# aperezhortal/pySPEEDY

Hardware: AMD Instinct MI355X
Metric: simulated-years/day (whole node), T30L8 (higher is better)
Workload: dtype f64

## Files before the change

### pyspeedy_amd/csrc/dyn_column.hpp

```cpp
#pragma once
#include <hip/hip_runtime.h>

#include "model.hpp"
#include "stream_store.hpp"
#include "vertical_consts.hpp"

namespace spd {

struct NoPrefetch {
    __device__ void operator()() const {}
};
template <bool STORE_ALL, typename F = NoPrefetch>
__device__ __forceinline__ void dyn_column(const ModelPtrs &P, const DynDeviceTables &D, int mem, int p, int j,
                                           double (&ttend)[KX], double (&trtend)[KX], double &utend_kx, double &vtend_kx,
                                           F before_products = F{}) {
    constexpr int NG = IX * IL;
    constexpr double AKAPd = 2.0f / 7.0f, RGASd = AKAPd * static_cast<double>(1004.0f);
    const size_t o3 = static_cast<size_t>(mem) * KX * NG + p, o2 = static_cast<size_t>(mem) * NG + p;
    double ug[KX], vg[KX], tg[KX], trg[KX], vorg[KX], divg[KX];
    const double cor = D.coriol[j];
#pragma unroll
    for (int k = 0; k < KX; ++k) {
        ug[k] = stream_load(&P.ug2[o3 + NG * k]);
        vg[k] = stream_load(&P.vg2[o3 + NG * k]);
        tg[k] = stream_load(&P.tg2[o3 + NG * k]);
        trg[k] = stream_load(&P.trg2[o3 + NG * k]);
        vorg[k] = stream_load(&P.vorg[o3 + NG * k]);
        divg[k] = stream_load(&P.divg[o3 + NG * k]);
    }
    const double px = stream_load(&P.px[o2]), py = stream_load(&P.py[o2]);
    __builtin_amdgcn_sched_barrier(0);
#pragma unroll
    for (int k = 0; k < KX; ++k) vorg[k] = vorg[k] + cor;
    double umean = 0.0, vmean = 0.0, dmean = 0.0;
#pragma unroll
    for (int k = 0; k < KX; ++k) {
// ... 20 lines not shown
    for (int k = 1; k < KX; ++k) temp[k] = sigdt[k] * (ug[k] - ug[k - 1]);
#pragma unroll
    for (int k = 0; k < KX; ++k) {
        const double v = vg[k] * vorg[k] - tgg[k] * RGASd * px - (temp[k + 1] + temp[k]) * vc::dhsr[k];
        if (STORE_ALL || k < KX - 1) stream_store(&P.utend[o3 + NG * k], v);
        if (k == KX - 1) utend_kx = v;
    }
#pragma unroll
    for (int k = 1; k < KX; ++k) temp[k] = sigdt[k] * (vg[k] - vg[k - 1]);
#pragma unroll
    for (int k = 0; k < KX; ++k) {
        const double v = -ug[k] * vorg[k] - tgg[k] * RGASd * py - (temp[k + 1] + temp[k]) * vc::dhsr[k];
        if (STORE_ALL || k < KX - 1) stream_store(&P.vtend[o3 + NG * k], v);
        if (k == KX - 1) vtend_kx = v;
    }
#pragma unroll
    for (int k = 1; k < KX; ++k) temp[k] = sigdt[k] * (tgg[k] - tgg[k - 1]) + sigm[k] * (vc::tref[k] - vc::tref[k - 1]);
#pragma unroll
    for (int k = 0; k < KX; ++k) {
        ttend[k] = tgg[k] * divg[k] - (temp[k + 1] + temp[k]) * vc::dhsr[k] + vc::fsgr[k] * tgg[k] * (sigdt[k + 1] + sigdt[k]) +
                   vc::tref3[k] * (sigm[k + 1] + sigm[k]) + AKAPd * (tg[k] * puv[k] - tgg[k] * dmean);
        if (STORE_ALL) stream_store(&P.ttend[o3 + NG * k], ttend[k]);
    }
#pragma unroll
    for (int k = 1; k < KX; ++k) temp[k] = sigdt[k] * (trg[k] - trg[k - 1]);
    temp[1] = 0.0;
    temp[2] = 0.0;
#pragma unroll
    for (int k = 0; k < KX; ++k) {
        trtend[k] = trg[k] * divg[k] - (temp[k + 1] + temp[k]) * vc::dhsr[k];
        if (STORE_ALL) stream_store(&P.trtend[o3 + NG * k], trtend[k]);
    }
    before_products();
#pragma unroll
    for (int k = 0; k < KX; ++k) {
        stream_store(&P.keg[o3 + NG * k], 0.5f * (ug[k] * ug[k] + vg[k] * vg[k]));
        stream_store(&P.utg[o3 + NG * k], -ug[k] * tgg[k]);
        stream_store(&P.vtg[o3 + NG * k], -vg[k] * tgg[k]);
        stream_store(&P.uqg[o3 + NG * k], -ug[k] * trg[k]);
        stream_store(&P.vqg[o3 + NG * k], -vg[k] * trg[k]);
    }
}

}
```

### pyspeedy_amd/csrc/model.hip

```cpp
#include <dlfcn.h>
#include <hip/hip_runtime.h>

#include <algorithm>
#include <atomic>
#include <chrono>
#include <cmath>
#include <cstring>
#include <map>
#include <memory>
#include <mutex>
#include <string>
#include <thread>
#include <utility>
#include <vector>

#include "model_state.hpp"
#include "coupler_point.hpp"
#include "diagnostics_block.hpp"
#include "bounded_call.hpp"
#include "launch_events.hpp"
#include "sppt_point.hpp"
#include "stream_apart.hpp"

namespace spd {
hipError_t run_spec2grid_table(const DeviceTables &T, const FieldDesc *table, int nfields, hipStream_t st);
hipError_t run_grid2spec_table(const DeviceTables &T, const FieldDesc *table, int nfields, hipStream_t st);
hipError_t run_physics(const DeviceTables &T, const spd_physics_args &a, int nmembers, int fp32, hipStream_t s);
hipError_t run_dyn_physics(const ModelPtrs &P, const DynDeviceTables &D, const DeviceTables &T, const spd_physics_args &a,
                           int first, int nmembers, int fp32, int store32, int diag, hipStream_t s);
hipError_t run_geopotential(const ModelPtrs &P, const DynDeviceTables &D, int first, int count, int tl, const SpptArgs *sppt,
                            int *rim, hipStream_t s);
hipError_t run_dyn_grid(const ModelPtrs &P, const DynDeviceTables &D, int M, hipStream_t s);
hipError_t run_spectral_step(const ModelPtrs &P, const DeviceTables &T, const DynDeviceTables &D, int M, int first, int count,
                             int j1, double dt, double eps, const CouplerArgs *cpl, bool early, int rim_mode, int *rim, hipStream_t s);
hipError_t run_diagnostics(const ModelPtrs &P, const DeviceTables &T, int M, int tl, int *err, double *diag, int ticket,
                           hipStream_t s);
hipError_t run_diagnostics_range(const ModelPtrs &P, const DeviceTables &T, int first, int count, int tl, int *err, double *diag,
                                 int ticket, hipStream_t s);
hipError_t run_coupler(const SurfacePtrs &S, int first, int count, const TimeInterp &w, int day, int land_coupling,
                       int sst_anomaly, int anom_planes, int fresh, hipStream_t s);
hipError_t run_forcing(const SurfacePtrs &S, int first, int count, const ZonalDevice &Z, double gamlat, double *corh_t,
                       double *corh_q, hipStream_t s);
hipError_t run_rest_state(const RestPtrs &R, int M, const RestConsts &c, hipStream_t s);
hipError_t run_scale_orog(const double *orog, double *phi0, long n, hipStream_t s);
hipError_t run_change_storage(double *array, long n, bool to_float, void *scratch, hipStream_t s);
hipError_t run_land_sea_init(const LandSeaPtrs &P, const LandSeaConsts &K, int first, int count, double *rows, hipStream_t s);
hipError_t run_multi_copy(const CopyList &L, hipStream_t s);
hipError_t run_spec2grid_table_check(const DeviceTables &T, const FieldDesc *table, int nfields, const CheckArgs &check, int members,
                                     hipStream_t st);
hipError_t run_copy_from_first(double *v, long n, int M, const int *flags, hipStream_t s);
hipError_t run_rest_surface(const double *phis0, double *forog, double *surf_ps, double *surf_q, const RestConsts &c, long n,
                            hipStream_t s);
hipError_t run_grid2spec(const DeviceTables &T, int stage, const double *src, double *dst, int prescale, int nfields,
                         hipStream_t stream);
// ... 143 lines not shown
    if (!m->inv_table32[0][0]) build_inverse_tables(m, false, true, m->inv_table32, batch);
    if (m->sppt_spec && !m->inv_table_sppt32[0][0]) build_inverse_tables(m, true, true, m->inv_table_sppt32, batch);
    return batch.upload(m);
}

static int build_tables(spd_model *m) {
    const int M = m->M;
    const ModelPtrs &P = m->P;
    auto spec = [](double *base, size_t field) { return base + field * NSPEC * C; };
    auto grid = [](double *base, size_t field) { return base + field * NG; };
    TableBatch batch;
    build_inverse_tables(m, false, false, m->inv_table, batch);
    auto pspec = [](double *base, size_t field) { return base + field * tri::kPacked * C; };
    constexpr int pk = kSpecPacked;
    std::vector<FieldDesc> t;
    t.reserve(static_cast<size_t>(M) * 73);
    const size_t pair = static_cast<size_t>(M) * 8;
    for (int i = 0; i < M; ++i) {
        const size_t w = static_cast<size_t>(i) * 8;
        for (int k = 0; k < 8; ++k) {
            t.push_back({grid(P.utend, w + k), pspec(P.specu, w + k), 1 | pk, 0});
            t.push_back({grid(P.vtend, w + k), pspec(P.specv, w + k), 1 | pk, 0});
            t.push_back({grid(P.utg, w + k), pspec(P.specu, pair + w + k), 1 | pk, 0});
            t.push_back({grid(P.vtg, w + k), pspec(P.specv, pair + w + k), 1 | pk, 0});
            t.push_back({grid(P.uqg, w + k), pspec(P.specu, 2 * pair + w + k), 1 | pk, 0});
            t.push_back({grid(P.vqg, w + k), pspec(P.specv, 2 * pair + w + k), 1 | pk, 0});
            t.push_back({grid(P.ttend, w + k), pspec(P.spec_tt, w + k), pk, 0});
            t.push_back({grid(P.trtend, w + k), pspec(P.spec_tr, w + k), pk, 0});
            t.push_back({grid(P.keg, w + k), pspec(P.spec_ke, w + k), pk, 0});
        }
        t.push_back({grid(P.psdtg, i), pspec(P.spec_ps, i), pk, 0});
    }
    batch.add(std::move(t), &m->fwd_table);
    for (int par = 0; par < 2; ++par) {
        std::vector<FieldDesc> ti, tf;
        const size_t half = static_cast<size_t>(M) * 16;
        for (int i = 0; i < M; ++i) {
            const size_t w = static_cast<size_t>(i) * 8, s1 = static_cast<size_t>(i) * 16;
            for (int k = 0; k < 8; ++k) {
                ti.push_back({spec(P.sv, s1 + k), grid(m->u_grid, w + k), 2, 0});
                ti.push_back({spec(P.sv, half + s1 + k), grid(m->v_grid, w + k), 2, 0});
                ti.push_back({spec(P.t, s1 + k), grid(m->t_grid, w + k), 1, 0});
                ti.push_back({spec(P.tr, s1 + k), grid(m->q_grid, w + k), 1, 0});
                ti.push_back({spec(m->phi_buf[par], w + k), grid(m->phi_grid, w + k), 1, 0});
                tf.push_back({grid(m->u_grid, w + k), spec(P.sv, s1 + k), 1, 0});
                tf.push_back({grid(m->v_grid, w + k), spec(P.sv, half + s1 + k), 1, 0});
                tf.push_back({grid(m->t_grid, w + k), spec(P.t, s1 + k), 0, 0});
                tf.push_back({grid(m->q_grid, w + k), spec(P.tr, s1 + k), 0, 0});
                tf.push_back({grid(m->phi_grid, w + k), spec(m->phi_buf[par], w + k), 0, 0});
            }
            ti.push_back({spec(P.ps, static_cast<size_t>(i) * 2), grid(m->ps_grid, i), 1, 0});
        }
        batch.add(std::move(ti), &m->exp_inv_table[par]);
        batch.add(std::move(tf), &m->exp_fwd_table[par]);
    }
    return batch.upload(m);
}

namespace spd {
int sample_ids(const char *who, const char *const *names, int n_names, std::vector<int> &ids) {
    if (n_names < 0 || (n_names > 0 && !names)) return m_fail(SPD_E_ARG, std::string(who) + ": bad list of variable names");
    for (int k = 0; k < n_names; ++k) {
        const int id = names[k] ? stats_id(names[k]) : -1;
        if (id < 0)
            return m_fail(SPD_E_ARG, std::string(who) + ": unknown variable '" + (names[k] ? names[k] : "(null)") +
                                         "' (u_grid, v_grid, t_grid, q_grid, phi_grid, ps_grid, precnv, precls, u_plev, v_plev, t_plev, "
// ... 514 lines not shown
        else (void)hipEventRecord(start, s);
    }
    ~ProfScope() {
        if (!stop) return;
        if (!attach) {
            (void)hipEventRecord(stop, s);
        } else if (pending_launch_events().start == start) {
            pending_launch_events() = LaunchEvents{};
            (void)hipEventRecord(start, s);
            (void)hipEventRecord(stop, s);
        }
    }
};

static bool folds(const spd_model *m) { return m->fold_geo && !m->nudge.loops(); }

static bool begin_step_geopotential(spd_model *m) {
    const bool fold = folds(m);
    const bool ahead = fold && m->phi_ahead;
    if (ahead) m->phi_cur ^= 1;
    m->P.phi = m->phi_buf[m->phi_cur];
    m->P.phi_next = fold ? m->phi_buf[m->phi_cur ^ 1] : nullptr;
    m->reg["phi"].ptr = m->P.phi;
    m->phi_ahead = fold;
    return !ahead;
}

static void sppt_advance(spd_model *m) {
    if (!m->sppt_on) return;
    m->sppt_first = false;
    m->sppt_step += 1;
}

static hipError_t step_range(spd_model *m, int j1, int j2, double dt, int compute_shortwave, int first, int count, int diag,
                             bool run_geo, const CouplerArgs *cpl, hipStream_t s, hipEvent_t after_grid2spec = nullptr,
                             const CheckArgs *ride = nullptr, int rim_mode = kRimPlain) {
    const DeviceTables &T = m->ctx->dev;
    const int M = m->M;
    hipError_t e = hipSuccess;
    if (m->fail_launch_after >= 0 && m->fail_launch_after-- == 0) return hipErrorLaunchFailure;
    SpptArgs sp{};
    if (m->sppt_on)
        sp = sppt_args(m->sppt_spec + static_cast<size_t>(first) * 8 * NSPEC * C, T, count, m->sppt_seed, m->sppt_member_base + first,
                       m->sppt_step, m->sppt_first ? 1 : 0);
    if (run_geo) {
        ProfScope ps(m, SPD_K_GEOPOTENTIAL, count, s);
        e = run_geopotential(m->P, m->D, first, count, 0, m->sppt_on ? &sp : nullptr, rim_mode == kRimSkip ? m->d_rim : nullptr,
                             s);
    } else if (m->sppt_on) {
        ProfScope ps(m, SPD_K_SPPT, 8 * count, s);
        e = run_sppt_update(sp, s);
    }
    spd_physics_args pa = m->pa;
    pa.compute_shortwave = compute_shortwave ? 1 : 0;
    pa.air_absortivity_co2 = m->air_absortivity_co2;
    pa.sppt_pattern = m->sppt_on ? m->sppt_grid : nullptr;
    if (e == hipSuccess) {
        const int per = m->inv_per_member + (m->sppt_on ? 8 : 0);
        FieldDesc *table = (m->stored32 ? (m->sppt_on ? m->inv_table_sppt32 : m->inv_table32)
                                         : (m->sppt_on ? m->inv_table_sppt : m->inv_table))[j2 - 1][m->phi_cur];
        ProfScope ps(m, SPD_K_SPEC2GRID, per * count, s);
        if (m->deferred.active && first == 0 && count == M && s == m->deferred.stream) {
            const int slot = m->deferred.slot;
            const CheckArgs chk{m->P.vor, m->P.div, m->P.t, m->deferred.time_level - 1, m->h_err[slot], m->d_diag, m->slot_ticket[slot]};
            e = run_spec2grid_table_check(T, table, per * count, chk, M, s);
            m->deferred.active = false;
            m->slot_rode[slot] = true;
            ++m->checks_rode;
        } else if (ride) {
            e = run_spec2grid_table_check(T, table + static_cast<size_t>(first) * per, per * count, *ride, count, s);
            ++m->checks_rode;
        } else {
            e = run_spec2grid_table(T, table + static_cast<size_t>(first) * per, per * count, s);
        }
    }
    if (e == hipSuccess) {
        if (m->split_dyn_physics && !m->phys_fp32) {
            {
                ProfScope ps(m, SPD_K_DYN_GRID, M, s);
                e = run_dyn_grid(m->P, m->D, M, s);
            }
            if (e == hipSuccess) {
                ProfScope ps(m, compute_shortwave ? SPD_K_PHYSICS_SW : SPD_K_PHYSICS, M, s);
                e = run_physics(T, pa, M, m->phys_fp32, s);
            }
        } else {
            ProfScope ps(m, compute_shortwave ? SPD_K_COLUMN_SW : SPD_K_COLUMN, count, s);
            e = run_dyn_physics(m->P, m->D, T, pa, first, count, m->phys_fp32, m->stored32 ? 1 : 0, diag, s);
        }
    }
    if (e == hipSuccess) {
        ProfScope ps(m, SPD_K_GRID2SPEC, 73 * count, s);
        e = run_grid2spec_table(T, m->fwd_table + static_cast<size_t>(first) * 73, 73 * count, s);
    }
    if (after_grid2spec && e == hipSuccess) e = hipEventRecord(after_grid2spec, s);
    const double eps = (j1 == 1) ? 0.0 : static_cast<double>(0.05f);
    if (e == hipSuccess) {
        ProfScope ps(m, SPD_K_SPECTRAL_STEP, count, s);
        const bool early = m->spectral_early < 0 ? count <= 8 : m->spectral_early != 0;
        e = run_spectral_step(m->P, T, m->D, M, first, count, j1 - 1, dt, eps, cpl, early, rim_mode, m->d_rim, s);
    }
    return e;
}

int spd_model_step_dynamics(spd_model_handle m, int j1, int j2, double dt, int compute_shortwave, void *stream) {
    if (!m) return m_fail(SPD_E_ARG, "spd_model_step_dynamics: null model");
    if (j1 < 1 || j1 > 2 || j2 < 1 || j2 > 2) return m_fail(SPD_E_ARG, "spd_model_step_dynamics: time levels are 1 or 2");
    if (!m->dyn) return m_fail(SPD_E_ARG, "spd_model_step_dynamics: call spd_model_set_time_step first");
    if (int rc = settle_deferred_check(m)) return rc;
    const bool run_geo = begin_step_geopotential(m);
    const hipError_t e = step_range(m, j1, j2, dt, compute_shortwave, 0, m->M, 1, run_geo, nullptr, static_cast<hipStream_t>(stream));
    if (e != hipSuccess) return m_fail(SPD_E_DEVICE, std::string("spd_model_step_dynamics: ") + hipGetErrorString(e));
    sppt_advance(m);
    return SPD_OK;
}

static int next_ticket(spd_model *m) {
    m->check_ticket = m->check_ticket % 0x0fffffff + 1;
    return m->check_ticket;
}

static int wait_codes(spd_model *m, const int *pinned, int ticket, hipEvent_t ev, hipStream_t s, int32_t *out, const char *who) {
    const volatile int *codes = pinned;
    const int M = m->M;
    auto all_there = [&]() {
        for (int i = 0; i < M; ++i)
// ... 798 lines not shown
        const long n = static_cast<long>(kv.second.bytes_member / sizeof(double)) * m->M;
        e = run_change_storage(static_cast<double *>(kv.second.ptr), n, fp32 != 0, scratch, nullptr);
        ++converted;
    }
    if (e == hipSuccess) e = hipDeviceSynchronize();
    (void)hipFree(scratch);
    if (e != hipSuccess) {
        if (converted > 0) {
            m->initialized = false;
            m->poisoned = std::string("a device error (") + hipGetErrorString(e) + ") interrupted the change of its fp32 / fp64 storage; "
                          "create and initialise a new model";
        }
        return m_fail(SPD_E_DEVICE, std::string("spd_model_set_physics_precision: ") + hipGetErrorString(e));
    }
    m->stored32 = want32;
    return SPD_OK;
}

int spd_model_set_physics_precision(spd_model_handle m, int fp32) {
    if (!m) return m_fail(SPD_E_ARG, "spd_model_set_physics_precision: null model");
    m->phys_fp32 = fp32 ? 1 : 0;
    return apply_storage(m, m->phys_fp32 && m->phys_store32);
}

int spd_model_get_option(spd_model_handle m, const char *name, int32_t *value) {
    if (!m || !name || !value) return m_fail(SPD_E_ARG, "spd_model_get_option: null argument");
    const std::string key(name);
    if (key == "diag_every_step") *value = m->diag_every_step ? 1 : 0;
    else if (key == "split_dyn") *value = m->split_dyn_physics ? 1 : 0;
    else if (key == "spectral_early") *value = m->spectral_early;
    else if (key == "member_groups") *value = m->nchunks;
    else if (key == "block_members") *value = m->block_members;
    else if (key == "physics_storage32") *value = m->phys_store32 ? 1 : 0;
    else if (key == "quiet_rim_members") {
        *value = -1;
        if (m->rim_call) {
            std::vector<int> flags(static_cast<size_t>(m->M));
            M_HIP(hipDeviceSynchronize());
            M_HIP(hipMemcpy(flags.data(), m->d_rim, sizeof(int) * flags.size(), hipMemcpyDeviceToHost));
            *value = 0;
            for (int f : flags) *value += f != 0 ? 1 : 0;
        }
    }
    else return m_fail(SPD_E_ARG, "spd_model_get_option: unknown option: " + key);
    return SPD_OK;
}

int spd_model_set_option(spd_model_handle m, const char *name, int32_t value) {
    if (!m || !name) return m_fail(SPD_E_ARG, "spd_model_set_option: null argument");
    const std::string key(name);
    const bool flag = value == 0 || value == 1;
    if (key == "diag_every_step" && flag) m->diag_every_step = value != 0;
    else if (key == "split_dyn" && flag) m->split_dyn_physics = value != 0;
    else if (key == "spectral_early" && value >= -1 && value <= 1) m->spectral_early = value;
    else if (key == "member_groups" && value >= 1 && value <= 4) m->nchunks = value < m->M ? value : m->M;
    else if (key == "block_members" && value >= 0) m->block_members = value;
    else if (key == "fail_launch_after" && value >= -1) m->fail_launch_after = value;
    else if (key == "prepare_multi_step" && value == 1) {
        if (int rc = ensure_steps_record(m, 360)) return rc;
        if (m->nchunks > 1 && !m->split_dyn_physics) return ensure_group_streams(m, m->nchunks);
    }
    else if (key == "physics_storage32" && flag) {
        m->phys_store32 = value != 0;
        return apply_storage(m, m->phys_fp32 && m->phys_store32);
    }
    else return m_fail(SPD_E_ARG, "spd_model_set_option: unknown option or value out of range: " + key);
// ... 366 lines not shown
```

### pyspeedy_amd/csrc/model_state.hpp

```cpp
#pragma once
#include <hip/hip_runtime.h>

#include <algorithm>
#include <cmath>
#include <cstring>
#include <map>
#include <memory>
#include <string>
#include <utility>
#include <vector>

#include "../../include/pyspeedy_amd.h"
#include "context.hpp"
#include "model.hpp"
#include "plev.hpp"
#include "stats.hpp"
#include "spectra.hpp"
#include "tape.hpp"
#include "enstape.hpp"
#include "acctape.hpp"
#include "nudge.hpp"
#include "breed.hpp"
#include "wintape.hpp"
#include "projtape.hpp"
// ... 1 lines not shown
#include "surface.hpp"

using namespace spd;

namespace spd {
constexpr int NG = IX * IL;
constexpr size_t C = 2;

struct RegEntry {
    void *ptr;
    size_t bytes_member;
    bool f32 = false;
};
}

struct spd_model {
    spd_context *ctx = nullptr;
    int M = 0;
    ModelPtrs P{};
    const spd_dyn_tables *dyn = nullptr;
    std::unique_ptr<spd_dyn_tables> dyn_private;
    DynDeviceTables D{};
    spd_physics_args pa{};
    struct Block {
        char *base;
        size_t size, used;
    };
    std::vector<Block> blocks;
    std::map<std::string, RegEntry> reg;
    FieldDesc *inv_table[2][2] = {{nullptr, nullptr}, {nullptr, nullptr}};
    FieldDesc *inv_table_sppt[2][2] = {{nullptr, nullptr}, {nullptr, nullptr}};
    FieldDesc *inv_table32[2][2] = {{nullptr, nullptr}, {nullptr, nullptr}}, *inv_table_sppt32[2][2] = {{nullptr, nullptr}, {nullptr, nullptr}};
    FieldDesc *fwd_table = nullptr;
    double *phi_buf[2] = {nullptr, nullptr};
    int phi_cur = 0;
    bool phi_ahead = false, fold_geo = true;
    bool groups_apart = true;
    int *d_err = nullptr;
    double *d_diag = nullptr;
    int *d_rim = nullptr;
    bool rim_call = false;
    int *h_err[2] = {nullptr, nullptr}, *h_err_sync = nullptr;
    hipEvent_t err_event[2] = {nullptr, nullptr};
    int next_slot = 0;
    bool slot_busy[2] = {false, false};
    int check_ticket = 0, slot_ticket[2] = {0, 0};
    struct DeferredCheck {
        bool active = false;
        int slot = -1, time_level = 2;
        hipStream_t stream = nullptr;
    } deferred;
    hipStream_t slot_stream[2] = {nullptr, nullptr};
    bool slot_rode[2] = {false, false};
    int checks_alone = 0, checks_rode = 0;
    double air_absortivity_co2 = 6.0;
    SurfacePtrs S{};
    Calendar cal;
    int current_step = 0;
    bool initialized = false;
    bool sppt_on = false, sppt_first = true;
    unsigned long long sppt_seed = 0;
    long long sppt_member_base = 0, sppt_step = 0;
    double *sppt_spec = nullptr, *sppt_grid = nullptr;
    int inv_per_member = 77;
    int nchunks = 1;
    int block_members = 32;
// ... 296 lines not shown
```

### pyspeedy_amd/csrc/transforms.hip

```cpp
#include <hip/hip_runtime.h>

#include "device_tables.hpp"
#include "diagnostics_block.hpp"
#include "launch_events.hpp"
#include "fft96.hpp"
#include "triangle.hpp"

namespace spd {

constexpr int kThreads = 512;
constexpr int kRowStride = 97;
constexpr int kRows = IL;
constexpr int kCStride = 63;
constexpr int kCBufDoubles = kRows * kCStride;
constexpr int kSpecPerLane = (NSPEC + kThreads - 1) / kThreads;
constexpr int kGridPerLane = (NGRID / 2 + kThreads - 1) / kThreads;
constexpr int kPlanePerLane = (kRows * MX + kThreads - 1) / kThreads;
constexpr int kHalfPlanePerLane = (IY * MX + kThreads - 1) / kThreads;
constexpr int kInvLanes = MX * 12;
constexpr size_t kLdsBytes = (kCBufDoubles + 2 * NSPEC) * sizeof(double);
static_assert(kRows * kRowStride <= kCBufDoubles + 2 * NSPEC, "R must fit inside C + S");

enum class Stage { Fused, LegendreOnly, FourierOnly };

using d2 = double __attribute__((ext_vector_type(2)));
using gd2_in = const __attribute__((address_space(1))) d2 *;
using gd2_out = __attribute__((address_space(1))) d2 *;
typedef float f2 __attribute__((ext_vector_type(2)));
using gf2_out = __attribute__((address_space(1))) f2 *;

__device__ inline int pos_re(int m) { return m == 0 ? 0 : 2 * m - 1; }
__device__ inline int pos_im(int m) { return m == 0 ? 61 : 2 * m; }

__device__ inline int wave_id() { return __builtin_amdgcn_readfirstlane(static_cast<int>(threadIdx.x) >> 6); }

#ifdef SPD_TRACE
__device__ unsigned long long spd_trace_acc[2][8];
__device__ unsigned long long spd_trace_cnt[2];
#define TRACE_BEGIN() unsigned long long trace_t0 = (threadIdx.x == 0) ? wall_clock64() : 0ull
// ... 168 lines not shown

    const bool as_float = (kcos & kGridAsFloat) != 0;
    kcos &= ~kGridAsFloat;
    gd2_out g = (gd2_out)dst;
    double cs[kGridPerLane];
#pragma unroll
    for (int it = 0; it < kGridPerLane; ++it) {
        const int idx = tid + it * kThreads;
        cs[it] = (kcos != 1 && idx < NGRID / 2) ? T.cosgr[idx / (IX / 2)] : 1.0;
    }
#pragma unroll
    for (int it = 0; it < kGridPerLane; ++it) {
        const int idx = tid + it * kThreads;
        if (idx < NGRID / 2) {
            const int r = idx / (IX / 2), ip = idx - r * (IX / 2);
            const double *a = rows + r * kRowStride + 2 * ip;
            d2 v{a[0], a[1]};
            if (kcos != 1) {
                v.x *= cs[it];
                v.y *= cs[it];
            }
            if (as_float) {
                const f2 w{static_cast<float>(v.x), static_cast<float>(v.y)};
                __builtin_nontemporal_store(w, &((gf2_out)dst)[idx]);
                continue;
            }
            __builtin_nontemporal_store(v, &g[idx]);
        }
    }
    TRACE_MARK(0, 4);
    TRACE_END(0);
}

template <Stage ST>
__device__ __forceinline__ void grid2spec_body(const double *__restrict__ src, double *__restrict__ dst,
                                               const DeviceTables &T, int prescale) {
    extern __shared__ __attribute__((aligned(16))) double lds[];
    double *rows = lds;
    double *cbuf = lds;
    d2 *s = reinterpret_cast<d2 *>(lds + kCBufDoubles);
    const int tid = threadIdx.x;
    const int wave = wave_id(), lane = tid & 63;
    const bool packed = ST == Stage::Fused && (prescale & kSpecPacked) != 0;
    prescale &= ~kSpecPacked;

    TRACE_BEGIN();
    if (ST == Stage::Fused) {
        gd2_in g = (gd2_in)src;
        constexpr int kPairTasks = IY * (IX / 2);
        constexpr int kPairPerLane = (kPairTasks + kThreads - 1) / kThreads;
        d2 gn[kPairPerLane], gs[kPairPerLane];
        double wj[kPairPerLane], cn[kPairPerLane], cs[kPairPerLane];
        const double *ctab = (prescale == 1) ? T.cosgr : T.cosgr2;
#pragma unroll
        for (int it = 0; it < kPairPerLane; ++it) {
            const int idx = tid + it * kThreads;
            if (idx < kPairTasks) {
                const int j = idx / (IX / 2), ip = idx - j * (IX / 2);
                gn[it] = __builtin_nontemporal_load(&g[(kRows - 1 - j) * (IX / 2) + ip]);
                gs[it] = __builtin_nontemporal_load(&g[j * (IX / 2) + ip]);
                wj[it] = T.wt[j];
                cn[it] = (prescale != 0) ? ctab[kRows - 1 - j] : 1.0;
                cs[it] = (prescale != 0) ? ctab[j] : 1.0;
            }
        }
#pragma unroll
        for (int it = 0; it < kPairPerLane; ++it) {
            const int idx = tid + it * kThreads;
            if (idx < kPairTasks) {
                const int j = idx / (IX / 2), ip = idx - j * (IX / 2);
                d2 n = gn[it], so = gs[it];
                if (prescale != 0) {
                    n.x *= cn[it];
                    n.y *= cn[it];
                    so.x *= cs[it];
                    so.y *= cs[it];
                }
                const double w = wj[it];
                double *an = rows + (kRows - 1 - j) * kRowStride + 2 * ip, *as = rows + j * kRowStride + 2 * ip;
                an[0] = (n.x + so.x) * w;
                an[1] = (n.y + so.y) * w;
                as[0] = (n.x - so.x) * w;
                as[1] = (n.y - so.y) * w;
            }
        }
    } else if (ST == Stage::FourierOnly) {
        gd2_in g = (gd2_in)src;
        d2 gv[kGridPerLane];
        double cs[kGridPerLane];
        const double *ctab = (prescale == 1) ? T.cosgr : T.cosgr2;
#pragma unroll
        for (int it = 0; it < kGridPerLane; ++it) {
            const int idx = tid + it * kThreads;
            if (idx < NGRID / 2) gv[it] = __builtin_nontemporal_load(&g[idx]);
            cs[it] = (prescale != 0 && idx < NGRID / 2) ? ctab[idx / (IX / 2)] : 1.0;
        }
#pragma unroll
        for (int it = 0; it < kGridPerLane; ++it) {
            const int idx = tid + it * kThreads;
            if (idx < NGRID / 2) {
                const int r = idx / (IX / 2), ip = idx - r * (IX / 2);
                d2 v = gv[it];
                if (prescale != 0) {
                    v.x *= cs[it];
                    v.y *= cs[it];
                }
                double *a = rows + r * kRowStride + 2 * ip;
                a[0] = v.x;
                a[1] = v.y;
            }
        }
    }
    if (ST != Stage::LegendreOnly) {
        __syncthreads();
        TRACE_MARK(1, 0);
        double *row = rows + lane * kRowStride;
// ... 114 lines not shown
                                                             DeviceTables T, int kcos) {
    const size_t f = blockIdx.x;
    constexpr size_t in = (ST == Stage::FourierOnly) ? NFOUR : 2 * NSPEC, out = (ST == Stage::LegendreOnly) ? NFOUR : NGRID;
    spec2grid_body<ST>(src + f * in, dst + f * out, T, kcos);
}

template <Stage ST>
__global__ __launch_bounds__(kThreads) void grid2spec_kernel(const double *__restrict__ src, double *__restrict__ dst,
                                                             DeviceTables T, int prescale) {
    const size_t f = blockIdx.x;
    constexpr size_t in = (ST == Stage::LegendreOnly) ? NFOUR : NGRID, out = (ST == Stage::FourierOnly) ? NFOUR : 2 * NSPEC;
    grid2spec_body<ST>(src + f * in, dst + f * out, T, prescale & ~kSpecPacked);
}

__global__ __launch_bounds__(kThreads) void spec2grid_table_kernel(const FieldDesc *__restrict__ table, DeviceTables T) {
    const FieldDesc e = table[blockIdx.x];
    spec2grid_body<Stage::Fused>(e.src, e.dst, T, e.flag, e.mode, e.src2);
}

static_assert(kThreads == 64 * KX, "a check block is a workgroup of the transform launch");
__global__ __launch_bounds__(kThreads, 8) void spec2grid_table_check_kernel(const FieldDesc *__restrict__ table, DeviceTables T,
                                                                            int members, CheckArgs check) {
    const int front = (members + 7) & ~7;
    if (static_cast<int>(blockIdx.x) < front) {
        if (static_cast<int>(blockIdx.x) < members) diagnostics_block<2>(check, T, check.first + static_cast<int>(blockIdx.x));
        return;
    }
    const FieldDesc e = table[blockIdx.x - front];
    spec2grid_body<Stage::Fused>(e.src, e.dst, T, e.flag, e.mode, e.src2);
}

__global__ __launch_bounds__(kThreads) void grid2spec_table_kernel(const FieldDesc *__restrict__ table, DeviceTables T) {
    const FieldDesc e = table[blockIdx.x];
    grid2spec_body<Stage::Fused>(e.src, e.dst, T, e.flag);
}

static hipError_t configure_once(const void *kernel, bool (&done)[64]) {
    int dev = 0;
    if (hipGetDevice(&dev) != hipSuccess || dev < 0 || dev >= 64) return hipErrorInvalidDevice;
    if (done[dev]) return hipSuccess;
    const hipError_t e = hipFuncSetAttribute(kernel, hipFuncAttributeMaxDynamicSharedMemorySize, static_cast<int>(kLdsBytes));
    done[dev] = e == hipSuccess;
    return e;
}
#define SPD_CONFIGURE(kernel)                                            \
    ([] {                                                                \
        static bool done[64] = {};                                       \
        return configure_once(reinterpret_cast<const void *>(kernel), done); \
    }())

template <Stage ST>
static hipError_t launch_s2g(const double *src, double *dst, const DeviceTables &T, int nfields, int kcos, hipStream_t st) {
    const hipError_t cfg = SPD_CONFIGURE(&spec2grid_kernel<ST>);
    if (cfg != hipSuccess) return cfg;
    hipLaunchKernelGGL((spec2grid_kernel<ST>), dim3(nfields), dim3(kThreads), kLdsBytes, st, src, dst, T, kcos);
    return hipGetLastError();
}

template <Stage ST>
static hipError_t launch_g2s(const double *src, double *dst, const DeviceTables &T, int nfields, int prescale,
                             hipStream_t st) {
    const hipError_t cfg = SPD_CONFIGURE(&grid2spec_kernel<ST>);
    if (cfg != hipSuccess) return cfg;
    hipLaunchKernelGGL((grid2spec_kernel<ST>), dim3(nfields), dim3(kThreads), kLdsBytes, st, src, dst, T, prescale);
    return hipGetLastError();
}

// ... 61 lines not shown
```

### pyspeedy_amd/model.py

```python
import ctypes as C

import numpy as np
import torch

from . import _lib
from ._lib import check
from .registry import REGISTRY

SHAPES = {n: (v.dtype, v.shape) for n, v in REGISTRY.items() if v.where == "device"}
SHAPES["sst_anom"] = (np.float64, (96, 48, 3))

DELT = 86400.0 / 36

KERNEL_NAMES = ("geopotential", "spec2grid", "column_sw", "column", "grid2spec", "spectral_step", "coupler", "forcing",
                "sppt", "dyn_grid", "physics_sw", "physics")

BC_MAP = (("orog", "orog"), ("fmask_orig", "lsm"), ("alb0", "alb"), ("veg_high", "vegh"), ("veg_low", "vegl"),
          ("stl12", "stl"), ("snowd12", "snowd"), ("soil_wc_l1", "swl1"), ("soil_wc_l2", "swl2"), ("soil_wc_l3", "swl3"),
          ("sst12", "sst"), ("sea_ice_frac12", "icec"))


class EnsembleModel:
    def __init__(self, spectral, nmembers):
        self.sp = spectral
# ... 157 lines not shown
        stream = C.c_void_p(torch.cuda.current_stream().cuda_stream)
        check(self._lib.spd_model_step_checked_begin(self._m, int(nsteps), stream), "spd_model_step_checked_begin")
        failed = np.zeros(self.nmembers, dtype=np.int32)
        accepted = np.zeros((self.nmembers, 7), dtype=np.int32)
        check(self._lib.spd_model_step_checked_end(self._m, failed.ctypes.data_as(C.POINTER(C.c_int32)),
                                                   accepted.ctypes.data_as(C.POINTER(C.c_int32))), "spd_model_step_checked_end")
        return failed, accepted

    @property
    def current_step(self):
        return int(self._lib.spd_model_current_step(self._m))

    @property
    def current_date(self):
        buf = (C.c_int * 5)()
        check(self._lib.spd_model_get_date(self._m, buf), "spd_model_get_date")
        return tuple(buf)

    def set_physics_precision(self, fp32):
        check(self._lib.spd_model_set_physics_precision(self._m, int(bool(fp32))), "spd_model_set_physics_precision")

    def memory(self):
        reserved, used = C.c_size_t(0), C.c_size_t(0)
        check(self._lib.spd_model_memory(self._m, C.byref(reserved), C.byref(used)), "spd_model_memory")
        return reserved.value, used.value

    def config(self):
        cfg = (C.c_int32 * 8)()
        check(self._lib.spd_model_get_config(self._m, cfg), "spd_model_get_config")
        created, apart = C.c_int32(0), C.c_int32(1)
        check(self._lib.spd_model_group_streams(self._m, C.byref(created), C.byref(apart)), "spd_model_group_streams")
        block = C.c_int32(0)
        check(self._lib.spd_model_get_option(self._m, b"block_members", C.byref(block)), "spd_model_get_option")
        streams, M = cfg[2], self.nmembers
        rounds = 1
        if block.value > 0 and M >= 4 * block.value and not cfg[3]:
            rounds = (M + max(streams, 1) * block.value - 1) // (max(streams, 1) * block.value)
        return dict(inv_per_member=cfg[0], diag_every_step=bool(cfg[1]), chunks=cfg[2], split_dyn=bool(cfg[3]),
                    fold_geo=bool(cfg[4]), coupler_in_spectral=bool(cfg[5]), physics_fp32=bool(cfg[6]),
                    physics_storage32=bool(cfg[7]), group_streams=created.value, group_streams_apart=bool(apart.value),
                    block_members=block.value, rounds=rounds)

    def set_option(self, name, value):
        rc = self._lib.spd_model_set_option(self._m, name.encode(), int(value))
        if rc == _lib.SPD_E_ARG:
            raise ValueError("unknown option or value out of range: %s = %r" % (name, value))
        check(rc, "spd_model_set_option")

    def get_option(self, name):
        value = C.c_int32(0)
        rc = self._lib.spd_model_get_option(self._m, name.encode(), C.byref(value))
        if rc == _lib.SPD_E_ARG:
            raise ValueError("unknown option: %s" % name)
        check(rc, "spd_model_get_option")
        return value.value

    def profile(self, level=1):
        check(self._lib.spd_model_profile(self._m, int(level)), "spd_model_profile")

    def profile_read_kernels(self):
        n = len(KERNEL_NAMES)
        mean, mn = np.zeros(n), np.zeros(n)
        cnt, units = np.zeros(n, dtype=np.int32), np.zeros(n, dtype=np.int32)
        check(self._lib.spd_model_profile_read_kernels(self._m, mean.ctypes.data_as(C.c_void_p), mn.ctypes.data_as(C.c_void_p),
                                                       cnt.ctypes.data_as(C.c_void_p), units.ctypes.data_as(C.c_void_p)),
              "spd_model_profile_read_kernels")
        return {KERNEL_NAMES[k]: (float(mean[k]), float(mn[k]), int(cnt[k]), int(units[k])) for k in range(n) if cnt[k]}

    def profile_read(self):
        ms, n, f = C.c_double(), C.c_int(), C.c_int()
        check(self._lib.spd_model_profile_read(self._m, C.byref(ms), C.byref(n), C.byref(f)), "spd_model_profile_read")
        return ms.value, n.value, f.value

    STATS_VARIABLES = ("u_grid", "v_grid", "t_grid", "q_grid", "phi_grid", "ps_grid", "precnv", "precls",
# ... 665 lines not shown
```

Before: 1.820 million.

## Compute nonlinear flux products inside grid2spec staging instead of storing them

Result: faster. 1.858 million, median of 6 (+2.1%).

```diff
diff --git a/pyspeedy_amd/csrc/dyn_column.hpp b/pyspeedy_amd/csrc/dyn_column.hpp
--- a/pyspeedy_amd/csrc/dyn_column.hpp
+++ b/pyspeedy_amd/csrc/dyn_column.hpp
@@ -2,6 +2,7 @@
 #include <hip/hip_runtime.h>
 
 #include "model.hpp"
+#include "staged_products.hpp"
 #include "stream_store.hpp"
 #include "vertical_consts.hpp"
 
@@ -88,13 +89,15 @@
         if (STORE_ALL) stream_store(&P.trtend[o3 + NG * k], trtend[k]);
     }
     before_products();
+    if (STORE_ALL) {
 #pragma unroll
-    for (int k = 0; k < KX; ++k) {
-        stream_store(&P.keg[o3 + NG * k], 0.5f * (ug[k] * ug[k] + vg[k] * vg[k]));
-        stream_store(&P.utg[o3 + NG * k], -ug[k] * tgg[k]);
-        stream_store(&P.vtg[o3 + NG * k], -vg[k] * tgg[k]);
-        stream_store(&P.uqg[o3 + NG * k], -ug[k] * trg[k]);
-        stream_store(&P.vqg[o3 + NG * k], -vg[k] * trg[k]);
+        for (int k = 0; k < KX; ++k) {
+            stream_store(&P.keg[o3 + NG * k], staged_product(kProdKe, ug[k], vg[k], 0.0));
+            stream_store(&P.utg[o3 + NG * k], staged_product(kProdFluxT, ug[k], tg[k], vc::tref[k]));
+            stream_store(&P.vtg[o3 + NG * k], staged_product(kProdFluxT, vg[k], tg[k], vc::tref[k]));
+            stream_store(&P.uqg[o3 + NG * k], staged_product(kProdFluxQ, ug[k], trg[k], 0.0));
+            stream_store(&P.vqg[o3 + NG * k], staged_product(kProdFluxQ, vg[k], trg[k], 0.0));
+        }
     }
 }
 
diff --git a/pyspeedy_amd/csrc/model.hip b/pyspeedy_amd/csrc/model.hip
--- a/pyspeedy_amd/csrc/model.hip
+++ b/pyspeedy_amd/csrc/model.hip
@@ -20,6 +20,7 @@
 #include "bounded_call.hpp"
 #include "launch_events.hpp"
 #include "sppt_point.hpp"
+#include "staged_products.hpp"
 #include "stream_apart.hpp"
 
 namespace spd {
@@ -229,6 +230,28 @@
         t.push_back({grid(P.psdtg, i), pspec(P.spec_ps, i), pk, 0});
     }
     batch.add(std::move(t), &m->fwd_table);
+    std::vector<FieldDesc> tp;
+    tp.reserve(static_cast<size_t>(M) * 73);
+    auto prod = [](int kind, int k) { return kind | (k << kProdLevelShift); };
+    for (int i = 0; i < M; ++i) {
+        const size_t w = static_cast<size_t>(i) * 8;
+        FieldDesc e[9][8];
+        for (int k = 0; k < 8; ++k) {
+            e[0][k] = {grid(P.utend, w + k), pspec(P.specu, w + k), 1 | pk, 0};
+            e[1][k] = {grid(P.vtend, w + k), pspec(P.specv, w + k), 1 | pk, 0};
+            e[2][k] = {grid(P.ttend, w + k), pspec(P.spec_tt, w + k), pk, 0};
+            e[3][k] = {grid(P.trtend, w + k), pspec(P.spec_tr, w + k), pk, 0};
+            e[4][k] = {grid(P.ug2, w + k), pspec(P.specu, pair + w + k), 1 | pk, prod(kProdFluxT, k), grid(P.tg2, w + k)};
+            e[5][k] = {grid(P.vg2, w + k), pspec(P.specv, pair + w + k), 1 | pk, prod(kProdFluxT, k), grid(P.tg2, w + k)};
+            e[6][k] = {grid(P.ug2, w + k), pspec(P.specu, 2 * pair + w + k), 1 | pk, prod(kProdFluxQ, k), grid(P.trg2, w + k)};
+            e[7][k] = {grid(P.vg2, w + k), pspec(P.specv, 2 * pair + w + k), 1 | pk, prod(kProdFluxQ, k), grid(P.trg2, w + k)};
+            e[8][k] = {grid(P.ug2, w + k), pspec(P.spec_ke, w + k), pk, prod(kProdKe, k), grid(P.vg2, w + k)};
+        }
+        for (int v = 0; v < 9; ++v)
+            for (int k = 0; k < 8; ++k) tp.push_back(e[v][k]);
+        tp.push_back({grid(P.psdtg, i), pspec(P.spec_ps, i), pk, 0});
+    }
+    batch.add(std::move(tp), &m->fwd_table_products);
     for (int par = 0; par < 2; ++par) {
         std::vector<FieldDesc> ti, tf;
         const size_t half = static_cast<size_t>(M) * 16;
@@ -809,6 +832,8 @@
     m->sppt_step += 1;
 }
 
+static bool staged_products(const spd_model *m) { return !(m->split_dyn_physics && !m->phys_fp32); }
+
 static hipError_t step_range(spd_model *m, int j1, int j2, double dt, int compute_shortwave, int first, int count, int diag,
                              bool run_geo, const CouplerArgs *cpl, hipStream_t s, hipEvent_t after_grid2spec = nullptr,
                              const CheckArgs *ride = nullptr, int rim_mode = kRimPlain) {
@@ -852,7 +877,7 @@
         }
     }
     if (e == hipSuccess) {
-        if (m->split_dyn_physics && !m->phys_fp32) {
+        if (!staged_products(m)) {
             {
                 ProfScope ps(m, SPD_K_DYN_GRID, M, s);
                 e = run_dyn_grid(m->P, m->D, M, s);
@@ -868,7 +893,8 @@
     }
     if (e == hipSuccess) {
         ProfScope ps(m, SPD_K_GRID2SPEC, 73 * count, s);
-        e = run_grid2spec_table(T, m->fwd_table + static_cast<size_t>(first) * 73, 73 * count, s);
+        const FieldDesc *fwd = staged_products(m) ? m->fwd_table_products : m->fwd_table;
+        e = run_grid2spec_table(T, fwd + static_cast<size_t>(first) * 73, 73 * count, s);
     }
     if (after_grid2spec && e == hipSuccess) e = hipEventRecord(after_grid2spec, s);
     const double eps = (j1 == 1) ? 0.0 : static_cast<double>(0.05f);
@@ -1733,6 +1759,7 @@
     else if (key == "member_groups") *value = m->nchunks;
     else if (key == "block_members") *value = m->block_members;
     else if (key == "physics_storage32") *value = m->phys_store32 ? 1 : 0;
+    else if (key == "staged_products") *value = staged_products(m) ? 1 : 0;
     else if (key == "quiet_rim_members") {
         *value = -1;
         if (m->rim_call) {
diff --git a/pyspeedy_amd/csrc/model_state.hpp b/pyspeedy_amd/csrc/model_state.hpp
--- a/pyspeedy_amd/csrc/model_state.hpp
+++ b/pyspeedy_amd/csrc/model_state.hpp
@@ -57,6 +57,7 @@
     FieldDesc *inv_table_sppt[2][2] = {{nullptr, nullptr}, {nullptr, nullptr}};
     FieldDesc *inv_table32[2][2] = {{nullptr, nullptr}, {nullptr, nullptr}}, *inv_table_sppt32[2][2] = {{nullptr, nullptr}, {nullptr, nullptr}};
     FieldDesc *fwd_table = nullptr;
+    FieldDesc *fwd_table_products = nullptr;
     double *phi_buf[2] = {nullptr, nullptr};
     int phi_cur = 0;
     bool phi_ahead = false, fold_geo = true;
diff --git a/pyspeedy_amd/csrc/staged_products.hpp b/pyspeedy_amd/csrc/staged_products.hpp
--- /dev/null
+++ b/pyspeedy_amd/csrc/staged_products.hpp
@@ -0,0 +1,18 @@
+#pragma once
+#include <hip/hip_runtime.h>
+
+namespace spd {
+
+constexpr int kProdNone = 0;
+constexpr int kProdFluxT = 1;
+constexpr int kProdFluxQ = 2;
+constexpr int kProdKe = 3;
+constexpr int kProdLevelShift = 8;
+
+__device__ __forceinline__ double staged_product(int kind, double a, double b, double tref) {
+    if (kind == kProdKe) return 0.5f * (a * a + b * b);
+    const double anomaly = b - tref;
+    return -a * anomaly;
+}
+
+}
diff --git a/pyspeedy_amd/csrc/transforms.hip b/pyspeedy_amd/csrc/transforms.hip
--- a/pyspeedy_amd/csrc/transforms.hip
+++ b/pyspeedy_amd/csrc/transforms.hip
@@ -4,7 +4,9 @@
 #include "diagnostics_block.hpp"
 #include "launch_events.hpp"
 #include "fft96.hpp"
+#include "staged_products.hpp"
 #include "triangle.hpp"
+#include "vertical_consts.hpp"
 
 namespace spd {
 
@@ -239,9 +241,71 @@
     TRACE_END(0);
 }
 
+__device__ __forceinline__ void stage_product_rows(double *lds, const double *__restrict__ src, const double *__restrict__ src2,
+                                                   const DeviceTables &T, int prescale, int mode) {
+    constexpr int kPairTasks = IY * (IX / 2);
+    constexpr int kPairPerLane = (kPairTasks + kThreads - 1) / kThreads;
+    const int tid = threadIdx.x;
+    double *rows = lds;
+    gd2_in g = (gd2_in)src;
+    const double *ctab = (prescale == 1) ? T.cosgr : T.cosgr2;
+    gd2_in gb = (gd2_in)src2;
+    const int kind = (mode & ((1 << kProdLevelShift) - 1)) == kProdKe ? kProdKe : kProdFluxT;
+    const double tref = (mode & ((1 << kProdLevelShift) - 1)) == kProdFluxT ? vc::tref[(mode >> kProdLevelShift) & (KX - 1)] : 0.0;
+    static_assert(kRows * kRowStride + IY + kRows <= kCBufDoubles + 2 * NSPEC, "wt and ctab fit behind the rows");
+    double *tab = lds + kRows * kRowStride;
+    double tv = 0.0;
+    if (tid < IY)
+        tv = T.wt[tid];
+    else if (tid < IY + kRows)
+        tv = ctab[tid - IY];
+    d2 an[kPairPerLane], as_[kPairPerLane], bn[kPairPerLane], bs[kPairPerLane];
+#pragma unroll
+    for (int it = 0; it < kPairPerLane; ++it) {
+        const unsigned idx = tid + it * kThreads;
+        if (idx < kPairTasks) {
+            const unsigned j = idx / (IX / 2), ip = idx - j * (IX / 2);
+            const unsigned in = (kRows - 1 - j) * (IX / 2) + ip, is = j * (IX / 2) + ip;
+            an[it] = __builtin_nontemporal_load(&g[in]);
+            as_[it] = __builtin_nontemporal_load(&g[is]);
+            bn[it] = __builtin_nontemporal_load(&gb[in]);
+            bs[it] = __builtin_nontemporal_load(&gb[is]);
+        }
+    }
+    __builtin_amdgcn_sched_barrier(0);
+    if (tid < IY + kRows) tab[tid] = tv;
+    __syncthreads();
+#pragma unroll
+    for (int it = 0; it < kPairPerLane; ++it) {
+        const int idx = tid + it * kThreads;
+        if (idx < kPairTasks) {
+            const int j = idx / (IX / 2), ip = idx - j * (IX / 2);
+            const double w = tab[j];
+            const double cn = (prescale != 0) ? tab[IY + kRows - 1 - j] : 1.0, cs = (prescale != 0) ? tab[IY + j] : 1.0;
+            d2 n, so;
+            n.x = staged_product(kind, an[it].x, bn[it].x, tref);
+            n.y = staged_product(kind, an[it].y, bn[it].y, tref);
+            so.x = staged_product(kind, as_[it].x, bs[it].x, tref);
+            so.y = staged_product(kind, as_[it].y, bs[it].y, tref);
+            if (prescale != 0) {
+                n.x *= cn;
+                n.y *= cn;
+                so.x *= cs;
+                so.y *= cs;
+            }
+            double *rn = rows + (kRows - 1 - j) * kRowStride + 2 * ip, *rs = rows + j * kRowStride + 2 * ip;
+            rn[0] = (n.x + so.x) * w;
+            rn[1] = (n.y + so.y) * w;
+            rs[0] = (n.x - so.x) * w;
+            rs[1] = (n.y - so.y) * w;
+        }
+    }
+}
+
 template <Stage ST>
 __device__ __forceinline__ void grid2spec_body(const double *__restrict__ src, double *__restrict__ dst,
-                                               const DeviceTables &T, int prescale) {
+                                               const DeviceTables &T, int prescale, int mode = 0,
+                                               const double *__restrict__ src2 = nullptr) {
     extern __shared__ __attribute__((aligned(16))) double lds[];
     double *rows = lds;
     double *cbuf = lds;
@@ -256,39 +320,43 @@
         gd2_in g = (gd2_in)src;
         constexpr int kPairTasks = IY * (IX / 2);
         constexpr int kPairPerLane = (kPairTasks + kThreads - 1) / kThreads;
-        d2 gn[kPairPerLane], gs[kPairPerLane];
-        double wj[kPairPerLane], cn[kPairPerLane], cs[kPairPerLane];
-        const double *ctab = (prescale == 1) ? T.cosgr : T.cosgr2;
-#pragma unroll
-        for (int it = 0; it < kPairPerLane; ++it) {
-            const int idx = tid + it * kThreads;
-            if (idx < kPairTasks) {
-                const int j = idx / (IX / 2), ip = idx - j * (IX / 2);
-                gn[it] = __builtin_nontemporal_load(&g[(kRows - 1 - j) * (IX / 2) + ip]);
-                gs[it] = __builtin_nontemporal_load(&g[j * (IX / 2) + ip]);
-                wj[it] = T.wt[j];
-                cn[it] = (prescale != 0) ? ctab[kRows - 1 - j] : 1.0;
-                cs[it] = (prescale != 0) ? ctab[j] : 1.0;
-            }
-        }
-#pragma unroll
-        for (int it = 0; it < kPairPerLane; ++it) {
-            const int idx = tid + it * kThreads;
-            if (idx < kPairTasks) {
-                const int j = idx / (IX / 2), ip = idx - j * (IX / 2);
-                d2 n = gn[it], so = gs[it];
-                if (prescale != 0) {
-                    n.x *= cn[it];
-                    n.y *= cn[it];
-                    so.x *= cs[it];
-                    so.y *= cs[it];
+        if (mode != kProdNone) {
+            stage_product_rows(lds, src, src2, T, prescale, mode);
+        } else {
+            d2 gn[kPairPerLane], gs[kPairPerLane];
+            double wj[kPairPerLane], cn[kPairPerLane], cs[kPairPerLane];
+            const double *ctab = (prescale == 1) ? T.cosgr : T.cosgr2;
+#pragma unroll
+            for (int it = 0; it < kPairPerLane; ++it) {
+                const int idx = tid + it * kThreads;
+                if (idx < kPairTasks) {
+                    const int j = idx / (IX / 2), ip = idx - j * (IX / 2);
+                    gn[it] = __builtin_nontemporal_load(&g[(kRows - 1 - j) * (IX / 2) + ip]);
+                    gs[it] = __builtin_nontemporal_load(&g[j * (IX / 2) + ip]);
+                    wj[it] = T.wt[j];
+                    cn[it] = (prescale != 0) ? ctab[kRows - 1 - j] : 1.0;
+                    cs[it] = (prescale != 0) ? ctab[j] : 1.0;
                 }
-                const double w = wj[it];
-                double *an = rows + (kRows - 1 - j) * kRowStride + 2 * ip, *as = rows + j * kRowStride + 2 * ip;
-                an[0] = (n.x + so.x) * w;
-                an[1] = (n.y + so.y) * w;
-                as[0] = (n.x - so.x) * w;
-                as[1] = (n.y - so.y) * w;
+            }
+#pragma unroll
+            for (int it = 0; it < kPairPerLane; ++it) {
+                const int idx = tid + it * kThreads;
+                if (idx < kPairTasks) {
+                    const int j = idx / (IX / 2), ip = idx - j * (IX / 2);
+                    d2 n = gn[it], so = gs[it];
+                    if (prescale != 0) {
+                        n.x *= cn[it];
+                        n.y *= cn[it];
+                        so.x *= cs[it];
+                        so.y *= cs[it];
+                    }
+                    const double w = wj[it];
+                    double *an = rows + (kRows - 1 - j) * kRowStride + 2 * ip, *as = rows + j * kRowStride + 2 * ip;
+                    an[0] = (n.x + so.x) * w;
+                    an[1] = (n.y + so.y) * w;
+                    as[0] = (n.x - so.x) * w;
+                    as[1] = (n.y - so.y) * w;
+                }
             }
         }
     } else if (ST == Stage::FourierOnly) {
@@ -469,7 +537,7 @@
 
 __global__ __launch_bounds__(kThreads) void grid2spec_table_kernel(const FieldDesc *__restrict__ table, DeviceTables T) {
     const FieldDesc e = table[blockIdx.x];
-    grid2spec_body<Stage::Fused>(e.src, e.dst, T, e.flag);
+    grid2spec_body<Stage::Fused>(e.src, e.dst, T, e.flag, e.mode, e.src2);
 }
 
 static hipError_t configure_once(const void *kernel, bool (&done)[64]) {
diff --git a/pyspeedy_amd/model.py b/pyspeedy_amd/model.py
--- a/pyspeedy_amd/model.py
+++ b/pyspeedy_amd/model.py
@@ -213,6 +213,10 @@
         check(self._lib.spd_model_group_streams(self._m, C.byref(created), C.byref(apart)), "spd_model_group_streams")
         block = C.c_int32(0)
         check(self._lib.spd_model_get_option(self._m, b"block_members", C.byref(block)), "spd_model_get_option")
+        staged = C.c_int32(0)
+        rc = self._lib.spd_model_get_option(self._m, b"staged_products", C.byref(staged))
+        if rc != _lib.SPD_E_ARG:
+            check(rc, "spd_model_get_option")
         streams, M = cfg[2], self.nmembers
         rounds = 1
         if block.value > 0 and M >= 4 * block.value and not cfg[3]:
@@ -220,7 +224,7 @@
         return dict(inv_per_member=cfg[0], diag_every_step=bool(cfg[1]), chunks=cfg[2], split_dyn=bool(cfg[3]),
                     fold_geo=bool(cfg[4]), coupler_in_spectral=bool(cfg[5]), physics_fp32=bool(cfg[6]),
                     physics_storage32=bool(cfg[7]), group_streams=created.value, group_streams_apart=bool(apart.value),
-                    block_members=block.value, rounds=rounds)
+                    block_members=block.value, rounds=rounds, forward_table="products" if staged.value else "plain")
 
     def set_option(self, name, value):
         rc = self._lib.spd_model_set_option(self._m, name.encode(), int(value))
```
